# XiaoshuiHuang/GMF

Hardware: AMD Instinct MI355X
Metric: correspondences/sec (whole node) (higher is better)
Workload: dtype f32 (split-fp16 MFMA operands, fp32 accumulate; the cross products of the attention's two contractions, S = K Q'^T and O = P V, on block-scaled e4m3 operands wherever the device-side score guard allows)

## Files before the change

gmf_amd/csrc/encoder_h2.hip:

```cpp
#include <algorithm>
#include <cstdlib>
#include "enc_common.hpp"
#include "enc_ff.hpp"
#include "launchers.hpp"

namespace gmf {

#ifndef GMF_H2_RING
#define GMF_H2_RING 2
#endif
constexpr int kRing = GMF_H2_RING;

template <int MODE>
GMF_DEVINL void front_h2_body(float* lds, const int bx, const int pair, const int zsel_in, const float* __restrict__ in,
                              const float* __restrict__ wst, const float* __restrict__ vecs, float* __restrict__ f_out,
                              float* __restrict__ q_out, float* __restrict__ k_out, float* __restrict__ v_out, int N, int tiles,
                              const PairTab* __restrict__ ptab = nullptr, unsigned* __restrict__ v_scale = nullptr,
                              const PvGuard guard = {}) {
  const int lane = threadIdx.x & 63, h = lane >> 5, i = lane & 31;
  const int wave = __builtin_amdgcn_readfirstlane(threadIdx.x >> 6);
  const size_t row0 = pair_row0(ptab, pair, N);
  N = pair_rows(ptab, pair, N);
  const int tiles_p = ptab ? (N + 31) >> 5 : tiles;
  if (bx * kWavesPerWG >= tiles_p) return;
// ... 19 lines not shown
    if (MODE == 1 || MODE == 3) {
      const int row = tile * 32 + i;
      float pk[4];
#pragma unroll
      for (int e = 0; e < 4; ++e) {
        const int k = 4 * h + e;
        pk[e] = (row < N && k < 6) ? in[(row0 + row) * 6 + k] : 0.f;
      }
      const float4* w0 = reinterpret_cast<const float4*>(vecs + 5 * C) + lane;
#pragma unroll
      for (int mb = 0; mb < 4; ++mb) {
        f32x16 acc = zero16();
        const float4 w = w0[mb * 64];
        acc = mfma32(w.x, pk[0], acc); acc = mfma32(w.y, pk[1], acc);
        acc = mfma32(w.z, pk[2], acc); acc = mfma32(w.w, pk[3], acc);
        float b[16];
        load_vec_block(b, vecs + 4 * C, mb, h);
#pragma unroll
        for (int r = 0; r < 16; ++r) x[16 * mb + r] = acc[r] + b[r];
      }
    } else {
      load_frag_p32<CF>(x, in + toff, lane);
    }
    if (MODE == 2) {
#pragma unroll
      for (int e = 0; e < CF; ++e) f[e] = x[e];
    } else {
      fx.set(x);
#pragma unroll
      for (int mb = 0; mb < 4; ++mb) {
        const f16x8* lw = as_h2(ss.acquire());
        f32x16 acc = zero16();
        mma_wx_h2<8>(acc, lw, fx);
        float b[16];
        load_vec_block(b, vecs, mb, h);
#pragma unroll
        for (int r = 0; r < 16; ++r) f[16 * mb + r] = relu_nan(fmaf(acc[r], kH2Inv, b[r]));
      }
    }
  }
  if (active && zsel <= 0 && MODE != 2) store_frag_p32<CF>(f_out + toff, f, lane);
  if (MODE == 3) {
    if (guard.stat_next && active) {
      float ssq = 0.f;
#pragma unroll
      for (int e = 0; e < CF; ++e) ssq = fmaf(f[e], f[e], ssq);
      pv_stat_raise(guard.stat_next, pair, ssq, tile * 32 + i < N, lane);
    }
    return;
  }
  fx.set(f);

  const bool v8 = pv_planes_on(v_scale, guard, pair);
  unsigned* const sw_tile = v_scale ? v_scale + ((size_t)pair * tiles + tile) * 128 + lane : nullptr;
  unsigned ksw = 0;
#pragma unroll
  for (int which = 0; which < 2; ++which) {
    if (zsplit && zsel != which) continue;
    float* dst = (which == 0 ? q_out : k_out) + toff;
#pragma unroll
    for (int mb = 0; mb < 4; ++mb) {
      const f16x8* lw = as_h2(ss.acquire());
      f32x16 acc = zero16();
      mma_wx_h2<8>(acc, lw, fx);
      float b[16], t[16];
      load_vec_block(b, vecs + (1 + which) * C, mb, h);
#pragma unroll
      for (int r = 0; r < 16; ++r) t[r] = fmaf(acc[r], kH2Inv, b[r]);
      if (active) {
        if (which == 1 && v8) store_block_v8(dst, mb, t, lane, ksw);
        else store_block_h2(dst, mb, t, lane);
      }
    }
    if (which == 1 && active && v8) sw_tile[64] = ksw;
  }
  if (zsplit && zsel != 2) return;
  unsigned vsw = 0;
#pragma unroll
  for (int db = 0; db < 4; ++db) {
    const f16x8* lw = as_h2(ss.acquire());
    f32x16 acc = zero16();
    mma_xw_h2<8>(acc, lw, fx);
    const float bv = vecs[3 * C + 32 * db + i];
    float t[16];
#pragma unroll
    for (int r = 0; r < 16; ++r) t[r] = fmaf(acc[r], kH2Inv, bv);
    if (active) {
      if (v8) store_block_v8(v_out + toff, db, t, lane, vsw);
      else store_block_h2(v_out + toff, db, t, lane);
    }
  }
  if (active && v8) sw_tile[0] = vsw;
}

template <int MODE>
__global__ void __launch_bounds__(256, 2)
k_front_h2(const float* __restrict__ in, const float* __restrict__ wst, const float* __restrict__ vecs,
           float* __restrict__ f_out, float* __restrict__ q_out, float* __restrict__ k_out,
           float* __restrict__ v_out, int N, int tiles, const PairTab* __restrict__ ptab, unsigned* __restrict__ v_scale,
           const PvGuard guard) {
  __shared__ __attribute__((aligned(16))) float lds[kRing * kStageFloats];
  front_h2_body<MODE>(lds, blockIdx.x, blockIdx.y, gridDim.z == 3 ? (int)blockIdx.z : -1, in, wst, vecs, f_out, q_out, k_out, v_out,
                      N, tiles, ptab, v_scale, guard);
}

GMF_DEVINL void load_frag_rowmajor(float (&x)[CF], const float* __restrict__ rows_base, int row, int n_rows, int h) {
  const float4* p = reinterpret_cast<const float4*>(rows_base + (size_t)min(row, n_rows - 1) * C) + h;
  const bool ok = row < n_rows;
#pragma unroll
  for (int g = 0; g < CF / 4; ++g) {
    const float4 t = p[8 * (g >> 2) + 2 * (g & 3)];
    x[4 * g + 0] = ok ? t.x : 0.f; x[4 * g + 1] = ok ? t.y : 0.f; x[4 * g + 2] = ok ? t.z : 0.f; x[4 * g + 3] = ok ? t.w : 0.f;
  }
}

template <bool PE, bool ROWMAJOR = false>
GMF_DEVINL void ctx_prep_h2_body(float* lds, const int bx, const int pair, const int set, const int nb, const float* __restrict__ ctx,
                                 const float* __restrict__ wst, const float* __restrict__ vecs, float* __restrict__ out, int T,
                                 int ttiles, int wst_stride, int vec_stride) {
  const int lane = threadIdx.x & 63, h = lane >> 5, i = lane & 31;
  const int wave = __builtin_amdgcn_readfirstlane(threadIdx.x >> 6);
  const int tile_raw = bx * kWavesPerWG + wave;
  const bool active = tile_raw < ttiles;
  const int tile = active ? tile_raw : ttiles - 1;
  wst += (size_t)set * wst_stride;
  vecs += (size_t)set * vec_stride;
  const float* pair_base = ROWMAJOR ? ctx + (size_t)pair * T * C : ctx + (size_t)pair * ttiles * (32 * C);
  float* dst = out + (((size_t)set * nb + pair) * ttiles + tile) * kStageFloats;

  StageStream ss;
  ss.init(lds, lds + kStageFloats, wave, kWavesPerWG, lane, wst, 4);
  ss.prime();
  FragH2<8> cx;
  {
    float x[CF], cn[CF];
    if (PE) lcpe_frag(x, pair_base, tile * 32 + i, T, vecs, h);
    else if (ROWMAJOR) load_frag_rowmajor(x, pair_base, tile * 32 + i, T, h);
    else load_frag_p32<CF>(x, pair_base + (size_t)tile * (32 * C), lane);
    layernorm_frag<CF>(cn, x, vecs + 4 * C, vecs + 5 * C, h);
    cx.set(cn);
  }
  f16x8* kdst = reinterpret_cast<f16x8*>(dst);
  f16x8* vdst = reinterpret_cast<f16x8*>(dst + 32 * DH);
#pragma unroll
  for (int mb = 0; mb < 2; ++mb) {
// ... 422 lines not shown
    fusion_ff_h2p_body<SPLIT>(lds, bx, r % nb, nb, r / nb, hs, x1, wst, vecs, x2_out, ttiles, part);
    return;
  }
  const int j = id - n_a;
  front_h2_body<3>(lds, j % gx_f, j / gx_f, -1, in, fwst, fvecs, f_out, q_out, k_out, v_out, N, tiles, ptab, nullptr, guard);
}

constexpr int kLinLdsFloats = 4 * kStageFloats + 7 * C + (3 * C + 2 * FFH) + kWavesPerWG * 2 * C + 3 * C;

template <int PART, int NP = 3, bool QSKIP = false>
GMF_DEVINL void linear_h2_body(float* lds, const float* __restrict__ f_in, const float* __restrict__ front_wst,
                               const float* __restrict__ front_vec, const float* __restrict__ ctx_img,
                               const float* __restrict__ attn_wst, const float* __restrict__ attn_vec,
                               const float* __restrict__ ff_wst, const float* __restrict__ ff_vec, float* __restrict__ q_out,
                               float* __restrict__ k_out, float* __restrict__ v_out, float* __restrict__ x2_out, int N, int tiles,
                               int T, int ttiles, const PairTab* __restrict__ ptab = nullptr,
                               unsigned* __restrict__ v_scale = nullptr,
                               const PvGuard guard = {}) {
  const int lane = threadIdx.x & 63, h = lane >> 5, i = lane & 31;
  const int wave = __builtin_amdgcn_readfirstlane(threadIdx.x >> 6);
  const int pair = blockIdx.y;
  if (ptab) N = ptab[pair].n;
  const int tiles_p = ptab ? (N + 31) >> 5 : tiles;
  if ((int)blockIdx.x * kWavesPerWG >= tiles_p) return;
  const int tile_raw = blockIdx.x * kWavesPerWG + wave;
  const bool active = tile_raw < tiles_p;
  const int tile = active ? tile_raw : tiles_p - 1;
  const float* pair_base = f_in + (size_t)pair * tiles * (32 * C);
  const size_t toff = ((size_t)pair * tiles + tile) * (32 * C);

  float* const lvec_a = lds + 4 * kStageFloats;
  float* const lvec_f = lvec_a + 7 * C;
  float* const halo = lvec_f + (3 * C + 2 * FFH) + wave * (2 * C);
  float* const lvec_p = lvec_f + (3 * C + 2 * FFH) + kWavesPerWG * (2 * C);
  if (PART != 2) dma_vec(front_vec + C, lvec_p, 3 * C, wave, kWavesPerWG, lane);
  if (PART != 1) {
    dma_vec(attn_vec, lvec_a, 7 * C, wave, kWavesPerWG, lane);
    dma_vec(ff_vec, lvec_f, 3 * C + 2 * FFH, wave, kWavesPerWG, lane);
    LcpeHalo<CF>::issue(pair_base, tile, tiles_p, halo, lane);
  }
  StageRing<4> ss;
  if (PART == 0) ss.init(lds, wave, lane, front_wst + (QSKIP ? 8 : 4) * kStageFloats, QSKIP ? 8 : 12, attn_wst, 2,
                         ctx_img + (size_t)pair * ttiles * kStageFloats, ttiles, attn_wst + 2 * kStageFloats, 2);
  else if (PART == 1) ss.init(lds, wave, lane, front_wst + 4 * kStageFloats, 12);
  else ss.init(lds, wave, lane, attn_wst, 2, ctx_img + (size_t)pair * ttiles * kStageFloats, ttiles, attn_wst + 2 * kStageFloats, 2);

  float f[CF];
  if (PART != 2) {
    FragH2<8> fx;
    load_frag_p32<CF>(f, f_in + toff, lane);
    fx.set(f);
    ss.prime();
    const bool v8 = pv_planes_on(v_scale, guard, pair);
    unsigned* const sw_tile = v_scale ? v_scale + ((size_t)pair * tiles + tile) * 128 + lane : nullptr;
    unsigned ksw = 0;
#pragma unroll
    for (int which = (QSKIP ? 1 : 0); which < 2; ++which) {
      float* dst = (which == 0 ? q_out : k_out) + toff;
#pragma unroll
      for (int mb = 0; mb < 4; ++mb) {
        constexpr int kYounger[4] = {8, 12, 16, 20};
        const int sidx = 4 * (which - (QSKIP ? 1 : 0)) + mb;
        const f16x8* lw = as_h2(PART == 1 ? ss.acquire()
                                : sidx == 0 ? ss.acquire_counted<kYounger[0]>() : sidx == 1 ? ss.acquire_counted<kYounger[1]>()
                                : sidx == 2 ? ss.acquire_counted<kYounger[2]>() : ss.acquire_counted<kYounger[3]>());
        f32x16 acc = zero16();
        mma_wx_h2n<8, NP>(acc, lw, fx);
        float t[16], bb[16];
        load_vec_block(bb, lvec_p + which * C, mb, h);
#pragma unroll
        for (int r = 0; r < 16; ++r) t[r] = fmaf(acc[r], kH2Inv, bb[r]);
        if (which == 1 && v8) store_block_v8(dst, mb, t, lane, ksw);
        else store_block_h2(dst, mb, t, lane);
      }
    }
    unsigned vsw = 0;
#pragma unroll
    for (int db = 0; db < 4; ++db) {
      const f16x8* lw = as_h2(PART == 1 ? ss.acquire() : ss.acquire_counted<20>());
      f32x16 acc = zero16();
      mma_xw_h2n<8, NP>(acc, lw, fx);
      float t[16];
      const float bvd = lvec_p[2 * C + 32 * db + i];
#pragma unroll
      for (int r = 0; r < 16; ++r) t[r] = fmaf(acc[r], kH2Inv, bvd);
      if (v8) store_block_v8(v_out + toff, db, t, lane, vsw);
      else store_block_h2(v_out + toff, db, t, lane);
    }
    if (v_scale) { sw_tile[0] = vsw; sw_tile[64] = ksw; }
  }

  if (PART == 1) {
    asm volatile("s_waitcnt vmcnt(0)" ::: "memory");
    return;
  }
  if (PART == 2) ss.prime();
  f32x16 x1a[4];
  {
    FragH2<4> qx;
    {
      float xp[CF];
      if (PART == 2) load_frag_p32<CF>(xp, f_in + toff, lane);
      else {
#pragma unroll
        for (int k = 0; k < CF; ++k) xp[k] = f[k];
      }
      if (PART == 2) {
        asm volatile("s_waitcnt vmcnt(0)" ::: "memory");
        __syncthreads();
      }
      LcpeHalo<CF>::apply(xp, halo, lvec_a, tile * 32 + i, N, lane);
      {
        FragH2<8> nx;
        {
          float xn[CF];
          layernorm_frag<CF>(xn, xp, lvec_a + 4 * C, lvec_a + 5 * C, h);
          nx.set(xn);
        }
#pragma unroll
        for (int mb = 0; mb < 2; ++mb) {
          const f16x8* lw = as_h2(ss.acquire());
          f32x16 acc = zero16();
          mma_wx_h2n<8, NP>(acc, lw, nx);
          float t[16];
#pragma unroll
          for (int r = 0; r < 16; ++r) t[r] = acc[r] * kH2Inv;
          qx.set_block(mb, t);
        }
      }
#pragma unroll
      for (int mb = 0; mb < 4; ++mb) {
        float b[16];
        load_vec_block(b, lvec_a + 6 * C, mb, h);
#pragma unroll
        for (int r = 0; r < 16; ++r) x1a[mb][r] = (xp[16 * mb + r] + b[r]) * 256.0f;
      }
    }
    f32x16 oacc[2];
    oacc[0] = zero16(); oacc[1] = zero16();
    float m_run = -INFINITY, l_half = 0.f;
    for (int t = 0; t < ttiles; ++t) {
      const f16x8* lk = as_h2(ss.acquire());
// ... 265 lines not shown
```

gmf_amd/csrc/encoder_kernels.hip:

```cpp
#include <algorithm>
#include <type_traits>
#include "enc_common.hpp"
#include "enc_ff.hpp"

namespace gmf {

template <int MODE>
__global__ void __launch_bounds__(256, 2)
k_front(const float* __restrict__ in, const float* __restrict__ wst, const float* __restrict__ vecs,
        float* __restrict__ f_out, float* __restrict__ q_out, float* __restrict__ k_out,
        float* __restrict__ v_out, int N, int tiles) {
  __shared__ __attribute__((aligned(16))) float lds[2 * kStageFloats];
  const int lane = threadIdx.x & 63, wave = threadIdx.x >> 6, h = lane >> 5, i = lane & 31;
  const int pair = blockIdx.y;
  const int tile_raw = blockIdx.x * kWavesPerWG + wave;
  const bool active = tile_raw < tiles;
  const int tile = active ? tile_raw : tiles - 1;
  const size_t toff = ((size_t)pair * tiles + tile) * (32 * C);

  constexpr bool FIRST = (MODE == 1);
  StageStream ss;
  if (MODE == 2) ss.init(lds, lds + kStageFloats, wave, kWavesPerWG, lane, wst + 4 * kStageFloats, 12);
  else ss.init(lds, lds + kStageFloats, wave, kWavesPerWG, lane, wst, 16);
  ss.prime();
// ... 486 lines not shown
#pragma unroll
        for (int r = 0; r < 16; ++r) t2[r] = relu_nan(fmaf(acc[r], kH2Inv, b[r]));
        m2x.set_block(mb, t2);
      }
    }
#pragma unroll
    for (int st = 0; st < 2; ++st) {
      const f16x8* lw = as_h2(ss.acquire());
#pragma unroll
      for (int hb = 0; hb < 2; ++hb) {
        if (!active) continue;
        const int mb = 2 * st + hb;
        f32x16 acc = zero16();
        mma_wx_h2<4>(acc, lw + hb * (2 * 4 * 64), m2x);
        float b[16], fz[16], tt[16];
        load_vec_block(b, vecs + 128, mb, h);
        fus_tile.load(fz, mb, lane, h);
#pragma unroll
        for (int r = 0; r < 16; ++r) tt[r] = fmaf(acc[r], kH2Inv, b[r]) + fz[r];
        if (NEXT_PCN) featx.set_block(mb, tt);
        else if (active) store_block_p32(out_tile, mb, tt, lane);
      }
    }
    if (NEXT_PCN) {
      float ssq = 0.f;
#pragma unroll
      for (int mb = 0; mb < 4; ++mb) {
        const f16x8* lw = as_h2(ss.acquire());
        if (!active) continue;
        f32x16 acc = zero16();
        mma_wx_h2<8>(acc, lw, featx);
        float b[16], tt[16];
        load_vec_block(b, next_bias, mb, h);
#pragma unroll
        for (int r = 0; r < 16; ++r) { tt[r] = relu_nan(fmaf(acc[r], kH2Inv, b[r])); ssq = fmaf(tt[r], tt[r], ssq); }
        store_block_p32(out_tile, mb, tt, lane);
      }
      if (stat_next && active) pv_stat_raise(stat_next, pair, ssq, row_valid, lane);
    }
}

struct AttnItem { int item, ks; bool split, valid; };
GMF_DEVINL AttnItem attn_item(int L, int n_items, int n_full, int ksplits) {
  const int chunk = n_items >> 3, rem = n_items & 7, xcd = L & 7, kth = L >> 3;
  const int start = (xcd < rem) ? xcd * (chunk + 1) : rem * (chunk + 1) + (xcd - rem) * chunk;
  const int items = chunk + (xcd < rem ? 1 : 0);
  const int nf = min(n_full, items);
  if (kth < nf) return AttnItem{start + kth, 0, false, true};
  const int j = kth - nf, r = j / ksplits;
  return AttnItem{start + nf + r, j - r * ksplits, true, nf + r < items};
}

constexpr float kInvU16 = 1.0f / 65535.0f;
template <int NPROD = 3, int CFMT = 0, int WAVES = 4, bool PVF8 = false>
GMF_DEVINL void scattn_h2p_body(float* lds, const int bid, const float* __restrict__ q_img, const float* __restrict__ k_img,
                                const float* __restrict__ v_img, const float* __restrict__ fus, const float* __restrict__ wst,
                                const float* __restrict__ vecs, float* out, int N, int tiles, int wgs_per_pair,
                                const float* __restrict__ c_dense, int n_items, int n_full, int ksplits,
                                float* __restrict__ part_o, float* __restrict__ part_ml, const float* __restrict__ next_wst,
                                const float* __restrict__ next_bias, const PairTab* __restrict__ ptab = nullptr,
                                const unsigned* __restrict__ v_scale = nullptr,
                                const float* qf_img = nullptr, const float* __restrict__ qw_wst = nullptr,
                                const float* __restrict__ qw_bias = nullptr,
                                unsigned* __restrict__ stat_next = nullptr) {
  static_assert(!PVF8 || NPROD == 3, "the fp8 cross products belong to the three-product form");
  float* const ldsK = lds;
  float* const ldsV = lds + 2 * kStageFloats;
  const int lane = threadIdx.x & 63, h = lane >> 5;
  const int wave = __builtin_amdgcn_readfirstlane(threadIdx.x >> 6);
  const unsigned lane_off16 = lane * 16;
  const AttnItem it = attn_item(bid, n_items, n_full, ksplits);
  if (!it.valid) return;
  const bool split = it.split;
  const int ks = it.ks;
  const int slot = it.item / wgs_per_pair, qblock = it.item - slot * wgs_per_pair;
  const int pair = ptab ? ptab[slot].ord : slot;
  if (ptab) N = ptab[pair].n;
  const int tiles_p = ptab ? (N + 31) >> 5 : tiles;
  if (qblock * WAVES >= tiles_p) return;
  const int t_begin = split ? (tiles_p * ks) / ksplits : 0;
  const int t_end = split ? (tiles_p * (ks + 1)) / ksplits : tiles_p;
  const int tile_raw = qblock * WAVES + wave;
  const bool active = tile_raw < tiles_p;
  const int tile = active ? tile_raw : tiles_p - 1;
  const size_t pbase = (size_t)pair * tiles;
  const size_t toff = (pbase + tile) * (32 * C);

  f16x8 qh[8], ql[8];
  if (NPROD == 3 && WAVES == 4 && qf_img) {
    FragH2<8> fx;
    {
      float fq[CF];
      load_frag_p32<CF>(fq, qf_img + toff, lane);
      fx.set(fq);
    }
#pragma unroll
    for (int st = 0; st < 4; ++st) dma_4k_s(qw_wst + st * kStageFloats + wave * 1024, lds + st * kStageFloats + wave * 1024, lane_off16);
    asm volatile("s_waitcnt vmcnt(0)" ::: "memory");
    __syncthreads();
#pragma unroll
    for (int mb = 0; mb < 4; ++mb) {
      const f16x8* lw = reinterpret_cast<const f16x8*>(lds + mb * kStageFloats) + lane;
      f32x16 acc = zero16();
      mma_wx_h2n<8, 3>(acc, lw, fx);
      float t[16], bq[16];
      load_vec_block(bq, qw_bias, mb, h);
#pragma unroll
      for (int r = 0; r < 16; ++r) t[r] = fmaf(acc[r], kH2Inv, bq[r]);
      split8h(&t[0], qh[2 * mb], ql[2 * mb]);
      split8h(&t[8], qh[2 * mb + 1], ql[2 * mb + 1]);
    }
    __syncthreads();
  } else {
    const f16x8* qp = reinterpret_cast<const f16x8*>(q_img + (pbase + tile) * (size_t)kStageFloats) + lane;
#pragma unroll
    for (int s = 0; s < 8; ++s) {
      qh[s] = qp[(0 * 8 + s) * 64];
      if (NPROD == 3) ql[s] = qp[(1 * 8 + s) * 64];
    }
  }
  i32x8 qb[4];
  unsigned qsw = 0;
  if (PVF8) {
#pragma unroll
    for (int cb = 0; cb < 4; ++cb) q_planes8(qh[2 * cb], ql[2 * cb], qh[2 * cb + 1], ql[2 * cb + 1], cb, lane, qb[cb], qsw);
  }
  constexpr int kCTile16 = CFMT ? 128 : 256;
  const f32x4* const crow = reinterpret_cast<const f32x4*>(c_dense) + ((pbase + tile) * (size_t)tiles) * kCTile16 + lane;
  float c[16];
  unsigned cw[8];
  const unsigned* const vsrow = PVF8 ? v_scale + pbase * 128 + lane : nullptr;
  unsigned vsw_next = 0, vsw = 0, ksw_next = 0, ksw = 0;
  const int psc = (lane & 32) ? 117 : 129;
  auto fetch_c = [&](int t) {
    const f32x4* ct = crow + (size_t)t * kCTile16;
    if (PVF8) {
      vsw_next = __builtin_nontemporal_load(vsrow + (size_t)t * 128);
      ksw_next = __builtin_nontemporal_load(vsrow + (size_t)min(t + 1, tiles_p - 1) * 128 + 64);
    }
    if (CFMT == 1) {
#pragma unroll
      for (int q2 = 0; q2 < 2; ++q2) {
        const f16x8 hv = __builtin_bit_cast(f16x8, __builtin_nontemporal_load(ct + q2 * 64));
#pragma unroll
        for (int e = 0; e < 8; ++e) c[8 * q2 + e] = (float)hv[e];
      }
    } else if (CFMT >= 2) {
#pragma unroll
      for (int q2 = 0; q2 < 2; ++q2) {
        const f32x4 v = __builtin_nontemporal_load(ct + q2 * 64);
#pragma unroll
        for (int e = 0; e < 4; ++e) cw[4 * q2 + e] = __float_as_uint(v[e]);
      }
    } else {
#pragma unroll
      for (int q = 0; q < 4; ++q) {
        const f32x4 v = __builtin_nontemporal_load(ct + q * 64);
        c[4 * q + 0] = v[0]; c[4 * q + 1] = v[1]; c[4 * q + 2] = v[2]; c[4 * q + 3] = v[3];
      }
    }
  };
  auto score = [&](int r, float sv) -> float {
    if (CFMT == 2) return (float)((r & 1) ? (cw[r >> 1] >> 16) : (cw[r >> 1] & 0xffffu)) * sv;
    return c[r] * sv;
  };
  auto expo = [&](float xv, float m_off) -> float {
    return __builtin_amdgcn_exp2f(CFMT == 2 ? fmaf(xv, kInvU16, -m_off) : xv - m_off);
  };
  auto mma_n = [&](f32x16& acc, f16x8 ah, f16x8 al, f16x8 bh, f16x8 bl) {
    if (NPROD == 3) mma3(acc, ah, al, bh, bl);
    else acc = mfma_h16(ah, bh, acc);
  };
  auto to_planes2 = [&](float x0, float x1, f16x8& hi, f16x8& lo, int j) {
    if (NPROD == 3) split2h(x0, x1, hi, lo, j);
    else { const f32x2 xx = {x0, x1}; const f16x2 hh = __builtin_convertvector(xx, f16x2); hi[j] = hh[0]; hi[j + 1] = hh[1]; }
  };
  auto planes_f8 = [&](const f16x8& hi, const f16x8& lo, const int j, const int kp, i32x8& pb, float& ls_h, float& ls_l) {
    const f16x2 hh = {hi[j], hi[j + 1]}, ll = {lo[j], lo[j + 1]};
    const f16x2 ones = {(_Float16)1.0f, (_Float16)1.0f};
    const int w = kp >> 1;
    if (kp & 1) {
      pb[w] = cvt2_fp8_f16<true>(pb[w], hh, 4.0f);
      pb[4 + w] = cvt2_fp8_f16<true>(pb[4 + w], ll, 0x1p-10f);
      ls_l = __builtin_amdgcn_fdot2(dec2_fp8_f16<true>(pb[4 + w], 0x1p-10f), ones, ls_l, false);
    } else {
      int d0, d1;
      asm("" : "=v"(d0), "=v"(d1));
      pb[w] = cvt2_fp8_f16<false>(d0, hh, 4.0f);
      pb[4 + w] = cvt2_fp8_f16<false>(d1, ll, 0x1p-10f);
      ls_l = __builtin_amdgcn_fdot2(dec2_fp8_f16<false>(pb[4 + w], 0x1p-10f), ones, ls_l, false);
    }
    ls_h = __builtin_amdgcn_fdot2(hh, ones, ls_h, false);
    asm volatile("" : "+v"(ls_h), "+v"(ls_l));
  };
  const float* gk = k_img + pbase * (size_t)kStageFloats;
  const float* gv = v_img + pbase * (size_t)kStageFloats;
  constexpr int kPiecesPerWave = ((NPROD == 3) ? 16 : 8) / WAVES;
  auto issue16k = [&](const float* g, float* l) {
#pragma unroll
    for (int q = 0; q < kPiecesPerWave; ++q) dma_piece_1k_s(g + (wave + WAVES * q) * 256, l + (wave + WAVES * q) * 256, lane_off16);
  };
  auto issueK = [&](int t) { issue16k(gk + (size_t)t * kStageFloats, ldsK + (t & 1) * kStageFloats); };
  auto issueV = [&](int t) { issue16k(gv + (size_t)t * kStageFloats, ldsV + (t & 1) * kStageFloats); };

  f32x16 oacc[4];
#pragma unroll
  for (int db = 0; db < 4; ++db) oacc[db] = zero16();
  float m_run = -INFINITY, l_half = 0.f;

  issueK(t_begin);
  if (t_begin + 1 < t_end) issueK(t_begin + 1);
  issueV(t_begin);
  fetch_c(t_begin);
  asm volatile("s_waitcnt vmcnt(0)" ::: "memory");
  __syncthreads();
  f32x16 s_a = zero16(), s_b;
  auto s_cross8 = [&](f32x16 acc, const f16x8* lkt, const int cb, const unsigned kscale) -> f32x16 {
    const i32x4* l8 = reinterpret_cast<const i32x4*>(lkt);
    const i32x4 a_lo = l8[(1 * 8 + 2 * cb) * 64], a_hi = l8[(1 * 8 + 2 * cb + 1) * 64];
    const i32x8 ka = {a_lo[0], a_lo[1], a_lo[2], a_lo[3], a_hi[0], a_hi[1], a_hi[2], a_hi[3]};
    return mfma_f8s2(ka, qb[cb], acc, cb, (int)kscale, (int)qsw);
  };
  if (active) {
    const f16x8* lk = reinterpret_cast<const f16x8*>(ldsK + (t_begin & 1) * kStageFloats) + lane;
    if (PVF8) {
      const unsigned ks0 = vsrow[(size_t)t_begin * 128 + 64];
#pragma unroll
      for (int s = 0; s < 8; ++s) s_a = mfma_h16(lk[(0 * 8 + s) * 64], qh[s], s_a);
#pragma unroll
      for (int cb = 0; cb < 4; ++cb) s_a = s_cross8(s_a, lk, cb, ks0);
    } else {
#pragma unroll
      for (int s = 0; s < 8; ++s) mma_n(s_a, lk[(0 * 8 + s) * 64], lk[(1 * 8 + s) * 64], qh[s], ql[s]);
    }
  }

  auto tile_top = [&](const int t, const f32x16& s_cur, float (&x)[16], float& mx) {
    asm volatile("s_waitcnt vmcnt(0)" ::: "memory");
    __syncthreads();
    if (PVF8) vsw = vsw_next;
#pragma unroll
    for (int r = 0; r < 16; r += 2) {
      x[r] = score(r, s_cur[r]);
      x[r + 1] = score(r + 1, s_cur[r + 1]);
      mx = __builtin_fmaxf(mx, __builtin_fmaxf(x[r], x[r + 1]));
    }
    __builtin_amdgcn_sched_barrier(0);
    if (t + 1 < t_end) fetch_c(t + 1);
    __builtin_amdgcn_sched_barrier(0);
  };
  auto issue_piece = [&](const int t, const int q) {
    if ((q & 3) >= kPiecesPerWave) return;
    if (q < 4) {
      if (t + 2 < t_end) dma_piece_1k_s(gk + (size_t)(t + 2) * kStageFloats + (wave + WAVES * q) * 256,
                                        ldsK + (t & 1) * kStageFloats + (wave + WAVES * q) * 256, lane_off16);
    } else {
      dma_piece_1k_s(gv + (size_t)(t + 1) * kStageFloats + (wave + WAVES * (q - 4)) * 256,
                     ldsV + ((t + 1) & 1) * kStageFloats + (wave + WAVES * (q - 4)) * 256, lane_off16);
    }
  };
  auto issue_k4 = [&](const int t) {
    if (WAVES == 4 && t + 2 < t_end && (NPROD == 3 || wave < 2))
      dma_4k_s(gk + (size_t)(t + 2) * kStageFloats + wave * 1024, ldsK + (t & 1) * kStageFloats + wave * 1024, lane_off16);
  };
  auto issue_v4 = [&](const int t) {
    if (WAVES == 4 && (NPROD == 3 || wave < 2))
      dma_4k_s(gv + (size_t)(t + 1) * kStageFloats + wave * 1024, ldsV + ((t + 1) & 1) * kStageFloats + wave * 1024, lane_off16);
  };
  auto rescale = [&](const bool moved, const float alpha) {
    if (__any(moved)) {
#pragma unroll
      for (int db = 0; db < 4; ++db)
#pragma unroll
        for (int r = 0; r < 16; ++r) oacc[db][r] *= alpha;
    }
  };
  auto tile_step = [&](const int t, const f32x16& s_cur, f32x16& s_next) {
    float x[16];
    float mx = -INFINITY, m_off = 0.f, alpha = 1.f, ls = 0.f;
    tile_top(t, s_cur, x, mx);
    const f16x8* lv = reinterpret_cast<const f16x8*>(ldsV + (t & 1) * kStageFloats) + lane;
    const f16x8* lk = reinterpret_cast<const f16x8*>(ldsK + ((t + 1) & 1) * kStageFloats) + lane;
    bool moved = false;
    f16x8 ph0, pl0, ph1, pl1;
    {
      mx = xhalf_max_swap(mx);
      if (CFMT == 2) mx *= kInvU16;
      const float m_new = __builtin_fmaxf(m_run, mx);
      moved = m_new > m_run;
      alpha = __builtin_amdgcn_exp2f(m_run - m_new);
      m_run = m_new;
      m_off = m_new - 10.0f;
      rescale(moved, alpha);
// ... 2 lines not shown
    {
      f16x8 kh = lk[0], kl = kh;
      if (NPROD == 3) kl = lk[8 * 64];
      f16x8 kh_n = kh, kl_n = kl;
#pragma unroll
      for (int u = 0; u < 24; ++u) {
        const int s = u / 3, pr = u % 3;
        if (pr == 0 && s < 7) { kh_n = lk[(0 * 8 + s + 1) * 64]; if (NPROD == 3) kl_n = lk[(1 * 8 + s + 1) * 64]; }
        if (NPROD == 3 || pr == 2) s_next = mma3_part(pr, s_next, kh, kl, qh[s], ql[s]);
        if (pr == 2) { kh = kh_n; kl = kl_n; }
        if (u < 2) {
        } else if (u <= 11) {
          const int r = u - 2;
          x[r] = expo(x[r], m_off);
          ls += x[r];
        } else if (u <= 15) {
          const int j = 2 * (u - 12);
          to_planes2(x[j], x[j + 1], ph0, pl0, j);
        } else if (u <= 21) {
          const int r = u - 6;
          x[r] = expo(x[r], m_off);
          ls += x[r];
        } else {
          const int j = 2 * (u - 22);
          to_planes2(x[8 + j], x[8 + j + 1], ph1, pl1, j);
        }
        __builtin_amdgcn_sched_barrier(0);
      }
    }
    {
      f16x8 vh = lv[0], vl = vh;
      if (NPROD == 3) vl = lv[8 * 64];
      f16x8 vh_n = vh, vl_n = vl;
#pragma unroll
      for (int u = 0; u < 24; ++u) {
        const int s2 = u / 12, db = (u % 12) / 3, pr = u % 3;
        if (pr == 0 && u < 21) {
          const int un = u + 3, slot = 2 * ((un % 12) / 3) + un / 12;
          vh_n = lv[(0 * 8 + slot) * 64]; if (NPROD == 3) vl_n = lv[(1 * 8 + slot) * 64];
        }
        if (NPROD == 3 || pr == 2) oacc[db] = mma3_part(pr, oacc[db], vh, vl, s2 ? ph1 : ph0, s2 ? pl1 : pl0);
        if (pr == 2) { vh = vh_n; vl = vl_n; }
        if (u < 2) {
          const int j = 4 + 2 * u;
          to_planes2(x[8 + j], x[8 + j + 1], ph1, pl1, j);
        }
        if (u >= 3 && u < 11) issue_piece(t, u - 3);
        __builtin_amdgcn_sched_barrier(0);
      }
    }
    l_half = fmaf(l_half, alpha, ls);
  };
  constexpr float kLazy = 5.0f;
  auto tile_step_f8 = [&](const int t, const f32x16& s_cur, f32x16& s_next) {
    float x[16];
    float mx = -INFINITY, m_off = 0.f, alpha = 1.f, ls = 0.f, ls_l = 0.f;
    asm volatile("s_waitcnt vmcnt(0)" ::: "memory");
    __syncthreads();
    vsw = vsw_next;
    ksw = ksw_next;
    const f16x8* lv = reinterpret_cast<const f16x8*>(ldsV + (t & 1) * kStageFloats) + lane;
    const f16x8* lk = reinterpret_cast<const f16x8*>(ldsK + ((t + 1) & 1) * kStageFloats) + lane;
    f16x8 ph0, pl0, ph1, pl1;
    i32x8 pb;
    f16x8 vr[3];
    auto hslot = [](int u) { return (0 * 8 + 2 * (u & 3) + (u >> 2)) * 64; };
    s_next = zero16();
    {
      const i32x4* lk8 = reinterpret_cast<const i32x4*>(lk);
      f16x8 kh = lk[0];
      f16x8 kh_n = kh;
      i32x4 k8a = lk8[(1 * 8) * 64], k8b = lk8[(1 * 8 + 1) * 64];
#pragma unroll
      for (int u = 0; u < 24; ++u) {
        const int s = u / 3, pr = u % 3;
        if (pr == 0 && s < 7) kh_n = lk[(0 * 8 + s + 1) * 64];
        if (pr == 2) s_next = mfma_h16(kh, qh[s], s_next);
        if (pr == 0 && (s & 1)) {
          const int cb = s >> 1;
          const i32x8 ka = {k8a[0], k8a[1], k8a[2], k8a[3], k8b[0], k8b[1], k8b[2], k8b[3]};
          s_next = mfma_f8s2(ka, qb[cb], s_next, cb, (int)ksw, (int)qsw);
          if (cb < 3) { k8a = lk8[(1 * 8 + 2 * cb + 2) * 64]; k8b = lk8[(1 * 8 + 2 * cb + 3) * 64]; }
        }
        if (pr == 2) kh = kh_n;
        if (u < 4) {
#pragma unroll
          for (int r = 4 * u; r < 4 * u + 4; r += 2) {
            x[r] = score(r, s_cur[r]);
            x[r + 1] = score(r + 1, s_cur[r + 1]);
            mx = __builtin_fmaxf(mx, __builtin_fmaxf(x[r], x[r + 1]));
          }
        }
        if (u == 3) {
          __builtin_amdgcn_sched_barrier(0);
          if (t + 1 < t_end) fetch_c(t + 1);
          __builtin_amdgcn_sched_barrier(0);
          mx = xhalf_max_swap(mx);
          if (CFMT == 2) mx *= kInvU16;
          const bool moved = mx > m_run + kLazy;
          const float m_new = moved ? mx : m_run;
          alpha = __builtin_amdgcn_exp2f(m_run - m_new);
          m_run = m_new;
          m_off = m_new - (10.0f - kLazy);
          rescale(moved, alpha);
        }
        if (u >= 4 && u < 20) x[u - 4] = expo(x[u - 4], m_off);
        if (u >= 6 && u <= 18 && (u & 1) == 0) {
          const int k = (u - 6) >> 1;
          if (k < 4) split2h(x[2 * k], x[2 * k + 1], ph0, pl0, 2 * k);
          else split2h(x[2 * k], x[2 * k + 1], ph1, pl1, 2 * k - 8);
        }
        if (u == 20) split2h(x[14], x[15], ph1, pl1, 6);
        if (u == 16) issue_k4(t);
        if (u == 23) issue_v4(t);
        if (u >= 21) vr[u - 21] = lv[hslot(u - 21)];
        __builtin_amdgcn_sched_barrier(0);
      }
    }
    {
      const i32x4* lv8 = reinterpret_cast<const i32x4*>(lv);
      i32x4 fa[2][2];
#pragma unroll
      for (int u = 0; u < 12; ++u) {
        if (u < 8) {
          const int s2 = u >> 2, db = u & 3;
          oacc[db] = mfma_h16(vr[u % 3], s2 ? ph1 : ph0, oacc[db]);
          if (u + 3 < 8) vr[u % 3] = lv[hslot(u + 3)];
          if (u == 4 || u == 6) { const int fd = (u - 4) >> 1; fa[fd][0] = lv8[(1 * 8 + 2 * fd) * 64]; fa[fd][1] = lv8[(1 * 8 + 2 * fd + 1) * 64]; }
          planes_f8(u < 4 ? ph0 : ph1, u < 4 ? pl0 : pl1, 2 * (u & 3), u, pb, ls, ls_l);
        } else {
          const int db = u - 8;
          const i32x4 a_lo = fa[db & 1][0], a_hi = fa[db & 1][1];
          const i32x8 va = {a_lo[0], a_lo[1], a_lo[2], a_lo[3], a_hi[0], a_hi[1], a_hi[2], a_hi[3]};
          oacc[db] = mfma_f8s(va, pb, oacc[db], db, (int)vsw, psc);
          if (db < 2) { fa[db & 1][0] = lv8[(1 * 8 + 2 * db + 4) * 64]; fa[db & 1][1] = lv8[(1 * 8 + 2 * db + 5) * 64]; }
        }
        __builtin_amdgcn_sched_barrier(0);
      }
    }
    l_half = fmaf(l_half, alpha, ls + ls_l);
  };
  auto tile_last = [&](const int t, const f32x16& s_cur) {
    float x[16];
    float mx = -INFINITY, ls = 0.f;
    tile_top(t, s_cur, x, mx);
    const f16x8* lv = reinterpret_cast<const f16x8*>(ldsV + (t & 1) * kStageFloats) + lane;
    const int jbase = t * 32 + 4 * h;
    mx = -INFINITY;
#pragma unroll
    for (int r = 0; r < 16; ++r) {
      const int jl = 8 * (r >> 2) + (r & 3);
      x[r] = (jbase + jl < N) ? x[r] : -INFINITY;
      mx = __builtin_fmaxf(mx, x[r]);
    }
    mx = xhalf_max_swap(mx);
    if (CFMT == 2) mx *= kInvU16;
    const float m_new = __builtin_fmaxf(m_run, mx);
    const bool moved = m_new > m_run;
    const float alpha = __builtin_amdgcn_exp2f(m_run - m_new);
    m_run = m_new;
    const float m_off = m_new - (PVF8 ? 10.0f - kLazy : 10.0f);
#pragma unroll
    for (int r = 0; r < 16; ++r) { x[r] = expo(x[r], m_off); if (!PVF8) ls += x[r]; }
    rescale(moved, alpha);
    if (PVF8) {
      i32x8 pb;
      float ls_l = 0.f;
#pragma unroll
      for (int s2 = 0; s2 < 2; ++s2) {
        f16x8 ph, pl;
        split8h(&x[8 * s2], ph, pl);
#pragma unroll
        for (int j = 0; j < 8; j += 2) planes_f8(ph, pl, j, 4 * s2 + (j >> 1), pb, ls, ls_l);
#pragma unroll
        for (int db = 0; db < 4; ++db) oacc[db] = mfma_h16(lv[(0 * 8 + 2 * db + s2) * 64], ph, oacc[db]);
      }
      ls += ls_l;
      const i32x4* lv8 = reinterpret_cast<const i32x4*>(lv);
#pragma unroll
      for (int db = 0; db < 4; ++db) {
        const i32x4 a_lo = lv8[(1 * 8 + 2 * db) * 64], a_hi = lv8[(1 * 8 + 2 * db + 1) * 64];
        const i32x8 va = {a_lo[0], a_lo[1], a_lo[2], a_lo[3], a_hi[0], a_hi[1], a_hi[2], a_hi[3]};
        oacc[db] = mfma_f8s(va, pb, oacc[db], db, (int)vsw, psc);
      }
    } else {
#pragma unroll
    for (int s2 = 0; s2 < 2; ++s2) {
      f16x8 ph, pl;
      split8h(&x[8 * s2], ph, pl);
#pragma unroll
      for (int db = 0; db < 4; ++db) {
        const int slot = 2 * db + s2;
        mma_n(oacc[db], lv[(0 * 8 + slot) * 64], lv[(1 * 8 + slot) * 64], ph, pl);
      }
    }
    }
    l_half = fmaf(l_half, alpha, ls);
  };
  if (!active) {
    for (int t = t_begin; t < t_end; ++t) {
      asm volatile("s_waitcnt vmcnt(0)" ::: "memory");
      __syncthreads();
      if (t + 1 < t_end) {
        if (PVF8) { issue_k4(t); issue_v4(t); }
        else {
#pragma unroll
          for (int q = 0; q < 8; ++q) issue_piece(t, q);
        }
      }
    }
  } else {
    int t = t_begin;
    if (PVF8) {
      for (; t + 2 < t_end; t += 2) {
        tile_step_f8(t, s_a, s_b);
        tile_step_f8(t + 1, s_b, s_a);
      }
      if (t + 1 < t_end) { tile_step_f8(t, s_a, s_b); tile_last(t + 1, s_b); }
      else tile_last(t, s_a);
    } else {
    for (; t + 2 < t_end; t += 2) {
      tile_step(t, s_a, s_b);
      tile_step(t + 1, s_b, s_a);
    }
    if (t + 1 < t_end) { tile_step(t, s_a, s_b); tile_last(t + 1, s_b); }
    else tile_last(t, s_a);
    }
  }
  if (split) {
    if (active) {
      float of[CF];
#pragma unroll
      for (int db = 0; db < 4; ++db)
#pragma unroll
        for (int r = 0; r < 16; ++r) of[16 * db + r] = oacc[db][r];
      const size_t n_tiles_all = (size_t)(n_items / wgs_per_pair) * tiles;
      const size_t pt = (size_t)ks * n_tiles_all + pbase + tile;
      store_frag_p32<CF>(part_o + pt * (32 * C), of, lane);
      const float lsum = xhalf_sum(l_half);
      if (h == 0) { part_ml[(pt * 32 + (lane & 31)) * 2] = m_run; part_ml[(pt * 32 + (lane & 31)) * 2 + 1] = lsum; }
    }
    return;
  }

  float o[CF];
  {
    const float inv = 1.0f / xhalf_sum(l_half);
#pragma unroll
    for (int db = 0; db < 4; ++db)
#pragma unroll
      for (int r = 0; r < 16; ++r) o[16 * db + r] = oacc[db][r] * inv;
  }
  __syncthreads();
  float* const lvec = lds + 2 * kStageFloats;
  stage_tail_vecs(lvec, vecs, next_wst ? next_bias : nullptr, wave, lane);
  StageStream ss;
  ss.init(lds, lds + kStageFloats, wave, WAVES, lane, wst, 5, next_wst, next_wst ? 4 : 0);
  ss.prime();
  const FusTile ft{fus + toff};
  if (next_wst) scattn_epilogue_h2<true>(o, active, ss, lvec, ft, out + toff, lane, h, lvec + 2 * C, stat_next, pair,
                                         tile_raw * 32 + (lane & 31) < N);
  else scattn_epilogue_h2<false>(o, active, ss, lvec, ft, out + toff, lane, h);
}

GMF_DEVINL bool attn_pv_on(const unsigned* __restrict__ v_scale, const PvGuard& guard, int bid, int n_items, int n_full, int ksplits,
                           int wgs_per_pair, const PairTab* __restrict__ ptab = nullptr) {
  if (!guard.stat) return v_scale != nullptr;
  const AttnItem it = attn_item(bid, n_items, n_full, ksplits);
  const int slot = it.valid ? it.item / wgs_per_pair : 0;
  return pv_planes_on(v_scale, guard, ptab ? ptab[slot].ord : slot);
}

// ... 1069 lines not shown
```

gmf_amd/csrc/gmf_api.cpp:

```cpp
#include "../../include/gmf_hip.h"

#include <hip/hip_runtime.h>

#include <cmath>
#include <cstdint>
#include <cstdio>
#include <algorithm>
#include <cstring>
#include <new>
#include <string>
#include <utility>
#include <vector>

#include "api_common.hpp"
#include "launchers_pose.hpp"
#include "launchers_solvers.hpp"
#include "launchers_spectral.hpp"
#include "launchers_pointcloud.hpp"
#include "launchers_sparse.hpp"
#include "launchers_dgr_input.hpp"
#include "launchers_correspondence.hpp"
#include "launchers_posegraph.hpp"

namespace {
// ... 623 lines not shown

static int encoder_forward_impl(gmf_handle* h, const gmf_encoder_weights* w, const float* corr_pos, const float* src_keypts,
                                const float* tgt_keypts, const float* p_tokens, const float* q_tokens, int B, int N, int T,
                                float* logits, float* feat_n, float* feat, gmf_stream_t stream, const int* n_points);

int gmf_encoder_forward(gmf_handle* h, const gmf_encoder_weights* w, const float* corr_pos, const float* src_keypts,
                        const float* tgt_keypts, const float* p_tokens, const float* q_tokens, int B, int N, int T,
                        float* logits, float* feat_n, float* feat, gmf_stream_t stream) {
  GMF_REQUIRE(h, GMF_ERR_BAD_ARG, "encoder_forward: null handle");
  GMF_REQUIRE(B > 0 && N > 0 && T > 0, GMF_ERR_UNSUPPORTED_SHAPE, "encoder_forward: empty input");
  return encoder_forward_impl(h, w, corr_pos, src_keypts, tgt_keypts, p_tokens, q_tokens, B, N, T, logits, feat_n, feat, stream, nullptr);
}

int gmf_encoder_forward_ragged(gmf_handle* h, const gmf_encoder_weights* w, const float* corr_pos, const float* src_keypts,
                               const float* tgt_keypts, const float* p_tokens, const float* q_tokens, const int* n_points, int B,
                               int T, float* logits, float* feat_n, float* feat, gmf_stream_t stream) {
  GMF_REQUIRE(h, GMF_ERR_BAD_ARG, "encoder_forward_ragged: null handle");
  GMF_REQUIRE(n_points, GMF_ERR_BAD_ARG, "encoder_forward_ragged: null n_points");
  GMF_REQUIRE(B > 0 && T > 0, GMF_ERR_UNSUPPORTED_SHAPE, "encoder_forward_ragged: empty input");
  return encoder_forward_impl(h, w, corr_pos, src_keypts, tgt_keypts, p_tokens, q_tokens, B, 0, T, logits, feat_n, feat, stream, n_points);
}

static int encoder_forward_impl(gmf_handle* h, const gmf_encoder_weights* w, const float* corr_pos, const float* src_keypts,
                                const float* tgt_keypts, const float* p_tokens, const float* q_tokens, int B, int N, int T,
                                float* logits, float* feat_n, float* feat, gmf_stream_t stream, const int* n_points) {
  if (int rc = check_weights(h, w)) return rc;
  GMF_REQUIRE(corr_pos && src_keypts && tgt_keypts && p_tokens && q_tokens && logits && feat_n, GMF_ERR_BAD_ARG,
              "encoder_forward: null pointer");
  SetDevice sd(h, stream);
  hipStream_t st = S(stream);
  const bool ragged = n_points != nullptr;
  int min_tiles = 0;
  if (ragged) {
    long long n_sum = 0;
    if (int rc = build_pair_table(h, n_points, B, -1.0, 0, &N, &n_sum, nullptr)) return rc;
    min_tiles = tiles_of(*std::min_element(n_points, n_points + B));
  }
  const int L = w->num_layers;
  const int tiles = tiles_of(N), tt = tiles_of(T);
  const EncoderPlan p = plan_encoder(h->tune, w, B, N, T, L, min_tiles, cu_count());
  GMF_REQUIRE(p.fused() || !ragged, GMF_ERR_UNSUPPORTED_SHAPE,
              "encoder_forward_ragged: ragged batches run on the default path only (split-fp16 weight images, at least two layers, the "
              "compat cache, \"fused_linear\" = 1, \"scattn_variant\" = 18)");
  const size_t act = p.act, tok = p.tok;
  gmf::PairTab* ptab;
  float *featA, *featB, *f, *q, *k, *v, *x1, *x2, *pts8, *pimg, *qimg, *f1ctx, *x1t, *imgfeat, *ctxall, *c_dense, *ff_part, *part_o,
      *part_ml;
  unsigned *v_scale, *fstat;
  if (int rc = arena_carve(h, {arena_buf(ptab, ragged ? (size_t)B : 0), arena_buf(featA, act), arena_buf(featB, act), arena_buf(f, act),
                               arena_buf(q, act), arena_buf(k, act), arena_buf(v, act), arena_buf(x1, act), arena_buf(x2, act),
                               arena_buf(pts8, (size_t)B * tiles * 32 * 8), arena_buf(pimg, tok), arena_buf(qimg, tok),
                               arena_buf(f1ctx, tok), arena_buf(x1t, tok), arena_buf(imgfeat, tok),
                               arena_buf(ctxall, (size_t)(L > 0 ? L : 1) * tok),
                               arena_buf(v_scale, (size_t)B * tiles * 128),
                               arena_buf(fstat, (size_t)(L + 1) * B * gmf::kPvStatStride),
                               arena_buf(c_dense, p.cache_floats),
                               arena_buf(ff_part, p.max_splits == 8 ? 8 * act : 0),
                               arena_buf(part_o, p.max_splits * act),
                               arena_buf(part_ml, (size_t)p.max_splits * B * tiles * 64)}))
    return rc;
  if (int rc = ragged ? upload_pair_table(h, ptab, B, st) : GMF_OK) return rc;
  gmf::CompatCache cc{c_dense, nullptr, part_o, part_ml};
  cc.half = p.half;
  cc.fmt = p.fmt;
  cc.ptab = ptab;
  cc.v_scale = p.v_fp8 ? v_scale : nullptr;
  unsigned* const zero_words = p.clear_stats ? fstat : nullptr;
  const int n_zero = p.clear_stats ? (L + 1) * B * gmf::kPvStatStride : 0;
  if (p.prologue) {
    GMF_HIP(gmf::launch_pro_ctx_pts(p_tokens, w->f1_ctx_wst_h2, w->f1_ctx_vec, f1ctx, B, T, tt, src_keypts, tgt_keypts, pts8, N, st, ptab,
                                    zero_words, n_zero));
    GMF_HIP(gmf::launch_pro_fattn_compat(q_tokens, f1ctx, w->f1_attn_wst_h2, w->f1_attn_vec, x1t, B, T, tt, pts8, c_dense, N, tiles,
                                         w->sigma_d, st, ptab));
    gmf::PvGuard g0;
    if (p.guard) g0.stat_next = fstat;
    GMF_HIP(gmf::launch_pro_ff_front(x1t, w->f1_ff_wst_h2, w->f1_ff_vec, imgfeat, B, tt, part_o, p.f1_ff_hs, corr_pos, w->front_wst_h2,
                                     w->front_vec, f, q, k, v, N, tiles, st, ptab, g0));
    if (p.f1_ff_hs > 1) GMF_HIP(gmf::launch_ff_reduce_h2(part_o, x1t, w->f1_ff_vec, imgfeat, B, tt, p.f1_ff_hs, st));
    GMF_HIP(gmf::launch_ctx_prep_h2(true, imgfeat, w->ctx_wst_h2, w->ctx_vec, ctxall, B, T, tt, L, w->ctx_wst_stride, w->ctx_vec_stride, st));
  } else {
    if (p.f1_h2) {
      GMF_HIP(gmf::launch_ctx_prep_h2(false, p_tokens, w->f1_ctx_wst_h2, w->f1_ctx_vec, f1ctx, B, T, tt, 1, 0, 0, st, true));
      GMF_HIP(gmf::launch_fusion_attn_h2(false, q_tokens, f1ctx, w->f1_attn_wst_h2, w->f1_attn_vec, x1t, B, T, tt, T, tt, st, true));
      GMF_HIP(gmf::launch_fusion_ff_h2(x1t, w->f1_ff_wst_h2, w->f1_ff_vec, imgfeat, B, tt, st, part_o, p.f1_ff_hs));
    } else {
      GMF_HIP(gmf::launch_pack_p32(p_tokens, pimg, B, T, kC, (long)T * kC, kC, 1, st));
      GMF_HIP(gmf::launch_pack_p32(q_tokens, qimg, B, T, kC, (long)T * kC, kC, 1, st));
      GMF_HIP(gmf::launch_ctx_prep(false, pimg, w->f1_ctx_wst, w->f1_ctx_vec, f1ctx, B, T, tt, 1, 0, 0, st));
      GMF_HIP(gmf::launch_fusion_attn(false, qimg, f1ctx, w->f1_attn_wst, w->f1_attn_vec, x1t, B, T, tt, T, tt, st));
      GMF_HIP(gmf::launch_fusion_ff(x1t, w->f1_ff_wst, w->f1_ff_vec, imgfeat, B, tt, st));
    }
    if (L > 0) {
      if (p.form != EncoderPlan::kFp32) GMF_HIP(gmf::launch_ctx_prep_h2(true, imgfeat, w->ctx_wst_h2, w->ctx_vec, ctxall, B, T, tt, L,
                                                                         w->ctx_wst_stride, w->ctx_vec_stride, st));
      else GMF_HIP(gmf::launch_ctx_prep(true, imgfeat, w->ctx_wst, w->ctx_vec, ctxall, B, T, tt, L, w->ctx_wst_stride,
                                        w->ctx_vec_stride, st));
    }
    GMF_HIP(gmf::launch_pack_pts8(src_keypts, tgt_keypts, pts8, B, N, st, ptab, zero_words, n_zero));
    if (p.cache) GMF_HIP(gmf::launch_compat_build(pts8, c_dense, B, N, tiles, w->sigma_d, p.fmt, st, ptab));
  }

  float* cur = featA;
  float* nxt = featB;
  if (p.fused()) {
    if (!p.prologue) {
      gmf::PvGuard g0;
      if (p.guard) g0.stat_next = fstat;
// ... 1209 lines not shown
```

gmf_amd/csrc/launchers.hpp:

```cpp
#pragma once
#include <hip/hip_runtime.h>

namespace gmf {

struct PairTab { int row0, n, S, k, ord, pad0, pad1, pad2; };

constexpr int kPvStatStride = 32;
struct PvGuard {
  const unsigned* stat = nullptr;
  const float* thr2 = nullptr;
  unsigned* stat_next = nullptr;
};

struct CompatCache {
  const float* dense;
  const float* tail_wst_h2;
  float* part_o;
  float* part_ml;
  const float* next_wst_h2 = nullptr;
  const float* next_bias = nullptr;
  bool half = false;
  const PairTab* ptab = nullptr;
  int fmt = 0;
  unsigned* v_scale = nullptr;
  const float* qf_img = nullptr;
  const float* qw_wst = nullptr;
  const float* qw_bias = nullptr;
  PvGuard guard;
};

struct Tuning {
  int scattn_variant = 18;
  bool use_cache = true;
  int key_splits = 0;
  bool tail_split = false;
  int ff_split = 0;
  bool front_split = true;
  bool wide_attn_tile = true;
  bool small_merge_tile = true;
  bool small_fattn_tile = true;
  bool small_roles = true;
  bool fused_linear = true;
  int conv_patch = 1;
  bool small_prologue = true;
  bool conv_small = true;
  int nms_binned = 1;
  bool topk_select = true;
  int mid_grid_roles = 512;
  bool q_in_attention = true;
  int pv_fp8 = 1;
  int compat_format = 0;
  int precision = 0;
  int spectral_col_splits = 0;
};

hipError_t launch_compat_build(const float* pts8, float* c_dense, int B, int N, int tiles, float sigma_d, int fmt, hipStream_t s,
                               const PairTab* ptab = nullptr);
hipError_t launch_front(int mode, const float* in, const float* wst, const float* vecs, float* f, float* q, float* k,
                        float* v, int B, int N, int tiles, hipStream_t s);
hipError_t launch_scattn_fp32(const float* q, const float* k, const float* v, const float* pts8, const float* fus,
                              const float* wst, const float* vecs, float* out, int B, int N, int tiles, float sigma_d,
                              hipStream_t s);
hipError_t launch_scattn_h2(const float* q, const float* k, const float* v, const float* pts8, const float* fus, const float* wst,
                            const float* vecs, float* out, int B, int N, int tiles, float sigma_d, hipStream_t s, const float* c_dense);
hipError_t launch_scattn_h2p(const float* q, const float* k, const float* v, const float* fus, const float* vecs, float* out, int B,
// ... 133 lines not shown
```

Before: 9.650 million.

## Pack per-tile fp8 V/K scale words into 16-byte records fetched once per tile pair

Result: no change. 9.672 million, median of 6 (+0.2%).

```diff
diff --git a/gmf_amd/csrc/encoder_h2.hip b/gmf_amd/csrc/encoder_h2.hip
--- a/gmf_amd/csrc/encoder_h2.hip
+++ b/gmf_amd/csrc/encoder_h2.hip
@@ -95,7 +95,7 @@
   fx.set(f);
 
   const bool v8 = pv_planes_on(v_scale, guard, pair);
-  unsigned* const sw_tile = v_scale ? v_scale + ((size_t)pair * tiles + tile) * 128 + lane : nullptr;
+  unsigned* const sw_pair = v_scale ? v_scale + (size_t)pair * sw_pair_words(tiles) : nullptr;
   unsigned ksw = 0;
 #pragma unroll
   for (int which = 0; which < 2; ++which) {
@@ -115,7 +115,7 @@
         else store_block_h2(dst, mb, t, lane);
       }
     }
-    if (which == 1 && active && v8) sw_tile[64] = ksw;
+    if (which == 1 && active && v8) sw_pair[sw_k_word(tile, lane)] = ksw;
   }
   if (zsplit && zsel != 2) return;
   unsigned vsw = 0;
@@ -133,7 +133,7 @@
       else store_block_h2(v_out + toff, db, t, lane);
     }
   }
-  if (active && v8) sw_tile[0] = vsw;
+  if (active && v8) sw_pair[sw_v_word(tile, lane)] = vsw;
 }
 
 template <int MODE>
@@ -662,7 +662,7 @@
     fx.set(f);
     ss.prime();
     const bool v8 = pv_planes_on(v_scale, guard, pair);
-    unsigned* const sw_tile = v_scale ? v_scale + ((size_t)pair * tiles + tile) * 128 + lane : nullptr;
+    unsigned* const sw_pair = v_scale ? v_scale + (size_t)pair * sw_pair_words(tiles) : nullptr;
     unsigned ksw = 0;
 #pragma unroll
     for (int which = (QSKIP ? 1 : 0); which < 2; ++which) {
@@ -697,7 +697,7 @@
       if (v8) store_block_v8(v_out + toff, db, t, lane, vsw);
       else store_block_h2(v_out + toff, db, t, lane);
     }
-    if (v_scale) { sw_tile[0] = vsw; sw_tile[64] = ksw; }
+    if (v_scale) { sw_pair[sw_v_word(tile, lane)] = vsw; sw_pair[sw_k_word(tile, lane)] = ksw; }
   }
 
   if (PART == 1) {
diff --git a/gmf_amd/csrc/encoder_kernels.hip b/gmf_amd/csrc/encoder_kernels.hip
--- a/gmf_amd/csrc/encoder_kernels.hip
+++ b/gmf_amd/csrc/encoder_kernels.hip
@@ -562,6 +562,7 @@
 }
 
 constexpr float kInvU16 = 1.0f / 65535.0f;
+template <bool ODD> struct TileHalf { static constexpr bool value = ODD; };
 template <int NPROD = 3, int CFMT = 0, int WAVES = 4, bool PVF8 = false>
 GMF_DEVINL void scattn_h2p_body(float* lds, const int bid, const float* __restrict__ q_img, const float* __restrict__ k_img,
                                 const float* __restrict__ v_img, const float* __restrict__ fus, const float* __restrict__ wst,
@@ -639,15 +640,16 @@
   const f32x4* const crow = reinterpret_cast<const f32x4*>(c_dense) + ((pbase + tile) * (size_t)tiles) * kCTile16 + lane;
   float c[16];
   unsigned cw[8];
-  const unsigned* const vsrow = PVF8 ? v_scale + pbase * 128 + lane : nullptr;
-  unsigned vsw_next = 0, vsw = 0, ksw_next = 0, ksw = 0;
+  const unsigned* const swrow = PVF8 ? v_scale + (size_t)pair * sw_pair_words(tiles) : nullptr;
+  unsigned sw_n0 = 0, sw_n1 = 0, sw_n2 = 0, sw_n3 = 0, sw_hv = 0, sw_hk = 0;
+  unsigned vsw = 0, ksw = 0;
   const int psc = (lane & 32) ? 117 : 129;
+  auto fetch_sw = [&](int t) {
+    const i32x4 r = __builtin_nontemporal_load(reinterpret_cast<const i32x4*>(swrow + sw_record(t >> 1, lane)));
+    sw_n0 = (unsigned)r[0]; sw_n1 = (unsigned)r[1]; sw_n2 = (unsigned)r[2]; sw_n3 = (unsigned)r[3];
+  };
   auto fetch_c = [&](int t) {
     const f32x4* ct = crow + (size_t)t * kCTile16;
-    if (PVF8) {
-      vsw_next = __builtin_nontemporal_load(vsrow + (size_t)t * 128);
-      ksw_next = __builtin_nontemporal_load(vsrow + (size_t)min(t + 1, tiles_p - 1) * 128 + 64);
-    }
     if (CFMT == 1) {
 #pragma unroll
       for (int q2 = 0; q2 < 2; ++q2) {
@@ -722,8 +724,10 @@
   if (t_begin + 1 < t_end) issueK(t_begin + 1);
   issueV(t_begin);
   fetch_c(t_begin);
+  if (PVF8) fetch_sw(t_begin);
   asm volatile("s_waitcnt vmcnt(0)" ::: "memory");
   __syncthreads();
+  if (PVF8) { sw_hv = sw_n2; sw_hk = sw_n3; }
   f32x16 s_a = zero16(), s_b;
   auto s_cross8 = [&](f32x16 acc, const f16x8* lkt, const int cb, const unsigned kscale) -> f32x16 {
     const i32x4* l8 = reinterpret_cast<const i32x4*>(lkt);
@@ -734,7 +738,7 @@
   if (active) {
     const f16x8* lk = reinterpret_cast<const f16x8*>(ldsK + (t_begin & 1) * kStageFloats) + lane;
     if (PVF8) {
-      const unsigned ks0 = vsrow[(size_t)t_begin * 128 + 64];
+      const unsigned ks0 = swrow[sw_k_word(t_begin, lane)];
 #pragma unroll
       for (int s = 0; s < 8; ++s) s_a = mfma_h16(lk[(0 * 8 + s) * 64], qh[s], s_a);
 #pragma unroll
@@ -748,7 +752,7 @@
   auto tile_top = [&](const int t, const f32x16& s_cur, float (&x)[16], float& mx) {
     asm volatile("s_waitcnt vmcnt(0)" ::: "memory");
     __syncthreads();
-    if (PVF8) vsw = vsw_next;
+    if (PVF8) vsw = (t & 1) ? sw_hv : sw_n0;
 #pragma unroll
     for (int r = 0; r < 16; r += 2) {
       x[r] = score(r, s_cur[r]);
@@ -857,13 +861,15 @@
     l_half = fmaf(l_half, alpha, ls);
   };
   constexpr float kLazy = 5.0f;
-  auto tile_step_f8 = [&](const int t, const f32x16& s_cur, f32x16& s_next) {
+  constexpr int kSwUnit = 22;
+  auto tile_step_f8 = [&](auto half, const int t, const f32x16& s_cur, f32x16& s_next) {
+    constexpr bool kOdd = decltype(half)::value;
     float x[16];
     float mx = -INFINITY, m_off = 0.f, alpha = 1.f, ls = 0.f, ls_l = 0.f;
     asm volatile("s_waitcnt vmcnt(0)" ::: "memory");
     __syncthreads();
-    vsw = vsw_next;
-    ksw = ksw_next;
+    if (kOdd) { vsw = sw_hv; ksw = sw_hk; }
+    else { vsw = sw_n0; ksw = sw_n1; sw_hv = sw_n2; sw_hk = sw_n3; }
     const f16x8* lv = reinterpret_cast<const f16x8*>(ldsV + (t & 1) * kStageFloats) + lane;
     const f16x8* lk = reinterpret_cast<const f16x8*>(ldsK + ((t + 1) & 1) * kStageFloats) + lane;
     f16x8 ph0, pl0, ph1, pl1;
@@ -916,6 +922,7 @@
           else split2h(x[2 * k], x[2 * k + 1], ph1, pl1, 2 * k - 8);
         }
         if (u == 20) split2h(x[14], x[15], ph1, pl1, 6);
+        if (kOdd && u == kSwUnit && t + 1 < t_end) fetch_sw(t + 1);
         if (u == 16) issue_k4(t);
         if (u == 23) issue_v4(t);
         if (u >= 21) vr[u - 21] = lv[hslot(u - 21)];
@@ -1017,12 +1024,19 @@
   } else {
     int t = t_begin;
     if (PVF8) {
-      for (; t + 2 < t_end; t += 2) {
-        tile_step_f8(t, s_a, s_b);
-        tile_step_f8(t + 1, s_b, s_a);
-      }
-      if (t + 1 < t_end) { tile_step_f8(t, s_a, s_b); tile_last(t + 1, s_b); }
-      else tile_last(t, s_a);
+      if ((t & 1) && t + 1 < t_end) {
+        tile_step_f8(TileHalf<true>{}, t, s_a, s_b);
+        s_a = s_b;
+        ++t;
+      }
+      if (!(t & 1)) {
+        for (; t + 2 < t_end; t += 2) {
+          tile_step_f8(TileHalf<false>{}, t, s_a, s_b);
+          tile_step_f8(TileHalf<true>{}, t + 1, s_b, s_a);
+        }
+        if (t + 1 < t_end) { tile_step_f8(TileHalf<false>{}, t, s_a, s_b); tile_last(t + 1, s_b); }
+        else tile_last(t, s_a);
+      } else tile_last(t, s_a);
     } else {
     for (; t + 2 < t_end; t += 2) {
       tile_step(t, s_a, s_b);
diff --git a/gmf_amd/csrc/gmf_api.cpp b/gmf_amd/csrc/gmf_api.cpp
--- a/gmf_amd/csrc/gmf_api.cpp
+++ b/gmf_amd/csrc/gmf_api.cpp
@@ -699,7 +699,7 @@
                                arena_buf(pts8, (size_t)B * tiles * 32 * 8), arena_buf(pimg, tok), arena_buf(qimg, tok),
                                arena_buf(f1ctx, tok), arena_buf(x1t, tok), arena_buf(imgfeat, tok),
                                arena_buf(ctxall, (size_t)(L > 0 ? L : 1) * tok),
-                               arena_buf(v_scale, (size_t)B * tiles * 128),
+                               arena_buf(v_scale, (size_t)B * gmf::sw_pair_words(tiles)),
                                arena_buf(fstat, (size_t)(L + 1) * B * gmf::kPvStatStride),
                                arena_buf(c_dense, p.cache_floats),
                                arena_buf(ff_part, p.max_splits == 8 ? 8 * act : 0),
diff --git a/gmf_amd/csrc/launchers.hpp b/gmf_amd/csrc/launchers.hpp
--- a/gmf_amd/csrc/launchers.hpp
+++ b/gmf_amd/csrc/launchers.hpp
@@ -11,6 +11,11 @@
   const float* thr2 = nullptr;
   unsigned* stat_next = nullptr;
 };
+
+constexpr size_t sw_pair_words(int tiles) { return 64 + (size_t)((tiles + 2) / 2) * 256; }
+constexpr size_t sw_record(int u, int lane) { return 64 + (size_t)u * 256 + 4 * lane; }
+constexpr size_t sw_v_word(int tile, int lane) { return sw_record(tile >> 1, lane) + 2 * (tile & 1); }
+constexpr size_t sw_k_word(int tile, int lane) { return tile ? sw_record((tile - 1) >> 1, lane) + 1 + 2 * ((tile - 1) & 1) : (size_t)lane; }
 
 struct CompatCache {
   const float* dense;
```
